# zhyever/Amodal-Depth-Anything

Hardware: AMD Instinct MI355X
Metric: images/sec at 518x518 bs=32 ViT-L (AmodalDAv2 forward) (higher is better)
Workload: dtype f16

## Files before the change

### amodal-depth-anything_amd/csrc/ada_attention.hip

```cpp
#include <stdlib.h>
#include <atomic>
#include <mutex>
#include <type_traits>
#include "ada_common.h"

namespace {

constexpr int HD = 64;
constexpr int QBLK = 128;
constexpr int KVB = 64;
constexpr int ROWB = 128;
constexpr int K_TILE = KVB * ROWB;
constexpr int V_TILE = KVB * ROWB;
constexpr int STAGE = K_TILE + V_TILE;

ADA_DEV void half_exchange(float x, float& lo, float& hi_) {
    unsigned a = __builtin_bit_cast(unsigned, x), b = a;
    asm volatile("s_nop 1\n\tv_permlane32_swap_b32 %0, %1" : "+v"(a), "+v"(b));
    lo = __builtin_bit_cast(float, a);
    hi_ = __builtin_bit_cast(float, b);
}

ADA_DEV float vmax3(float a, float b, float c) {
    float d;
    asm("v_max3_f32 %0, %1, %2, %3" : "=v"(d) : "v"(a), "v"(b), "v"(c));
    return d;
}
ADA_DEV float vmax2(float a, float b) {
    float d;
    asm("v_max_f32 %0, %1, %2" : "=v"(d) : "v"(a), "v"(b));
    return d;
}

struct RowSum {
    float a0 = 0.0f, a1 = 0.0f;
    ADA_DEV void add(float e0, float e1, opx2, bool) {
        a0 += e0;
        a1 += e1;
    }
    ADA_DEV float total() const { return a0 + a1; }
};

__global__ __launch_bounds__(256, 2) void attention_kernel_v3(const op_t* __restrict__ qkv, op_t* __restrict__ out, long ld_out,
                                                           int n_tok, int heads, int nqb, int n_bh) {
    __shared__ __attribute__((aligned(16))) char smem[2 * STAGE];

    const int tid = threadIdx.x;
    const int lane = tid & 63;
    const int wave = __builtin_amdgcn_readfirstlane(tid >> 6);
    const int l31 = lane & 31;
    const int hi = lane >> 5;

    int bh, qb;
    {
        const int nblk = gridDim.x, bid = blockIdx.x;
        const int q = nblk >> 3, r = nblk & 7;
        const int xcd = bid & 7, idx = bid >> 3;
        const int logical = (xcd < r ? xcd * (q + 1) : r * (q + 1) + (xcd - r) * q) + idx;
        bh = logical / nqb;
        qb = logical - bh * nqb;
    }
    const int b = bh / heads, h = bh - b * heads;
    const long D = (long)heads * HD;
    const long row_stride = 3 * D;
    const op_t* base = qkv + (long)b * n_tok * row_stride + (long)h * HD;
    const op_t* qptr = base;
    const op_t* kptr = base + D;
    const op_t* vptr = base + 2 * D;

    const int q_row = qb * QBLK + wave * 32 + l31;
    const int q_ld = q_row < n_tok ? q_row : n_tok - 1;
    const bool wave_active = (qb * QBLK + wave * 32) < n_tok;
    opx8 qf[4];
#pragma unroll
    for (int s = 0; s < 4; ++s) qf[s] = *(const opx8*)(qptr + (long)q_ld * row_stride + 16 * s + 8 * hi);

    const int srow = tid >> 3;
    const int sc = tid & 7;
    const int k_src_chunk = sc ^ ((srow >> 1) & 7);
    const int v_src_chunk = sc ^ (((srow >> 1) & 1) << 2);
    auto stage = [&](int buf, int t) {
        char* dst = smem + buf * STAGE + wave * 1024;
#pragma unroll
        for (int it = 0; it < 2; ++it) {
            int key = t * KVB + it * 32 + srow;
            if (key >= n_tok) key = n_tok - 1;
            const long off = (long)key * row_stride;
            __builtin_amdgcn_global_load_lds((const __attribute__((address_space(1))) void*)(kptr + off + k_src_chunk * 8),
                                             (__attribute__((address_space(3))) void*)(dst + it * 4096), 16, 0, 0);
            __builtin_amdgcn_global_load_lds((const __attribute__((address_space(1))) void*)(vptr + off + v_src_chunk * 8),
                                             (__attribute__((address_space(3))) void*)(dst + K_TILE + it * 4096), 16, 0, 0);
        }
    };

    f32x16 o[2];
#pragma unroll
    for (int db = 0; db < 2; ++db)
#pragma unroll
        for (int r = 0; r < 16; ++r) o[db][r] = 0.0f;
    float m_run = 0.0f, l_run = 0.0f;
    constexpr float RESCALE_THR = 8.0f;

    opx8 kx, qx;
#pragma unroll
    for (int j = 0; j < 8; ++j) { kx[j] = (op_t)0.0f; qx[j] = (op_t)0.0f; }
    if (hi == 0) kx[0] = (op_t)1.0f;

    const unsigned lds0 = (unsigned)(size_t)smem;
    const int swz = (l31 >> 1) & 7;
    unsigned kofs[4];
#pragma unroll
    for (int s = 0; s < 4; ++s) kofs[s] = l31 * ROWB + (((2 * s + hi) ^ swz) * 16);
    const int i16 = lane & 15;
    const int g1 = (lane >> 4) & 1;
    const int vsw = (i16 >> 3) & 1;
    const unsigned v_row_part = (4 * hi + (i16 >> 2)) * ROWB + (16 * g1 + 4 * (i16 & 3)) * 2;
    const unsigned vofs[2] = {v_row_part + (vsw ? 64u : 0u), v_row_part + (vsw ? 0u : 64u)};

    const int nt = (n_tok + KVB - 1) / KVB;
    stage(0, 0);
    asm volatile("s_waitcnt vmcnt(0)" ::: "memory");
    __syncthreads();

    for (int t = 0; t < nt; ++t) {
        const int cur = t & 1;
        if (t + 1 < nt) stage(cur ^ 1, t + 1);
        const unsigned kbase_l = lds0 + cur * STAGE;
        const unsigned vbase0 = kbase_l + K_TILE + vofs[0], vbase1 = kbase_l + K_TILE + vofs[1];

        if (wave_active) {
        opx8 kf[2][4];
#pragma unroll
        for (int kb = 0; kb < 2; ++kb)
#pragma unroll
            for (int s = 0; s < 4; ++s)
                asm volatile("ds_read_b128 %0, %1 offset:%2" : "=v"(kf[kb][s]) : "v"(kbase_l + kofs[s]), "i"(kb * 32 * ROWB));
        asm volatile("s_waitcnt lgkmcnt(0)" ::: "memory");
        __builtin_amdgcn_sched_barrier(0);
        f32x16 sT[2];
#pragma unroll
        for (int kb = 0; kb < 2; ++kb) {
#pragma unroll
            for (int r = 0; r < 16; ++r) sT[kb][r] = 0.0f;
            sT[kb] = mfma32(kx, qx, sT[kb]);
#pragma unroll
            for (int s = 0; s < 4; ++s) sT[kb] = mfma32(kf[kb][s], qf[s], sT[kb]);
        }
        __builtin_amdgcn_sched_barrier(0);
        opx4 vlo[2][2][2], vhi[2][2][2];
#pragma unroll
        for (int kb = 0; kb < 2; ++kb)
#pragma unroll
            for (int s = 0; s < 2; ++s) {
                asm volatile("ds_read_b64_tr_b16 %0, %1 offset:%2" : "=v"(vlo[kb][s][0]) : "v"(vbase0), "i"((kb * 32 + s * 16) * ROWB));
                asm volatile("ds_read_b64_tr_b16 %0, %1 offset:%2" : "=v"(vhi[kb][s][0]) : "v"(vbase0), "i"((kb * 32 + s * 16 + 8) * ROWB));
                asm volatile("ds_read_b64_tr_b16 %0, %1 offset:%2" : "=v"(vlo[kb][s][1]) : "v"(vbase1), "i"((kb * 32 + s * 16) * ROWB));
                asm volatile("ds_read_b64_tr_b16 %0, %1 offset:%2" : "=v"(vhi[kb][s][1]) : "v"(vbase1), "i"((kb * 32 + s * 16 + 8) * ROWB));
            }
        if (t == nt - 1) {
            const int kv0 = t * KVB;
#pragma unroll
            for (int kb = 0; kb < 2; ++kb)
#pragma unroll
                for (int r = 0; r < 16; ++r)
                    if (kv0 + kb * 32 + crow32(r, hi) >= n_tok) sT[kb][r] = -INFINITY;
        }

        float mx = sT[0][0];
#pragma unroll
        for (int kb = 0; kb < 2; ++kb)
#pragma unroll
            for (int r = 0; r < 16; ++r) mx = __builtin_fmaxf(mx, sT[kb][r]);
        {
            float a, b2;
            half_exchange(mx, a, b2);
            mx = __builtin_fmaxf(a, b2);
        }
        if (t == 0 || __any(mx > RESCALE_THR)) {
            const bool mv = (t == 0) || (mx > RESCALE_THR);
            const op_t m16 = (op_t)(m_run + mx);
            const float m_new = mv ? (float)m16 : m_run;
            const float delta = m_new - m_run;
            const float alpha = __builtin_amdgcn_fmed3f(__builtin_amdgcn_exp2f(-delta), 0.0f, 1.0f);
            l_run *= alpha;
            m_run = m_new;
            if (hi == 0) qx[0] = (op_t)(-m_new);
#pragma unroll
            for (int db = 0; db < 2; ++db)
#pragma unroll
                for (int r = 0; r < 16; ++r) o[db][r] *= alpha;
#pragma unroll
            for (int kb = 0; kb < 2; ++kb)
#pragma unroll
                for (int r = 0; r < 16; ++r) sT[kb][r] -= delta;
        }
        opx8 pf[2][2];
        RowSum rs;
#pragma unroll
        for (int kb = 0; kb < 2; ++kb) {
#pragma unroll
            for (int r = 0; r < 16; r += 2) {
                opx2 pp;
                const float e0 = __builtin_amdgcn_exp2f(sT[kb][r]), e1 = __builtin_amdgcn_exp2f(sT[kb][r + 1]);
                pp[0] = (op_t)e0;
                pp[1] = (op_t)e1;
                pf[kb][r >> 3][r & 7] = pp[0];
                pf[kb][r >> 3][(r & 7) + 1] = pp[1];
                rs.add(e0, e1, pp, (r & 2) != 0);
            }
        }
        l_run += rs.total();

        asm volatile("s_waitcnt lgkmcnt(0)" ::: "memory");
        __builtin_amdgcn_sched_barrier(0);
#pragma unroll
        for (int kb = 0; kb < 2; ++kb) {
#pragma unroll
            for (int s = 0; s < 2; ++s) {
#pragma unroll
                for (int db = 0; db < 2; ++db) {
                    const opx4 lo = vlo[kb][s][db], hi4 = vhi[kb][s][db];
                    opx8 vf;
                    vf[0] = lo[0]; vf[1] = lo[1]; vf[2] = lo[2]; vf[3] = lo[3];
                    vf[4] = hi4[0]; vf[5] = hi4[1]; vf[6] = hi4[2]; vf[7] = hi4[3];
                    o[db] = mfma32(vf, pf[kb][s], o[db]);
                }
            }
        }
        __builtin_amdgcn_sched_barrier(0);
        }

        asm volatile("s_waitcnt vmcnt(0)" ::: "memory");
        __syncthreads();
    }

    float l_lo, l_hi;
    half_exchange(l_run, l_lo, l_hi);
    const float inv = 1.0f / (l_lo + l_hi);
    if (q_row < n_tok) {
        op_t* orow = out + ((long)b * n_tok + q_row) * ld_out + (long)h * HD;
#pragma unroll
        for (int db = 0; db < 2; ++db) {
#pragma unroll
            for (int g = 0; g < 4; ++g) {
                opx4 v4;
#pragma unroll
                for (int e = 0; e < 4; ++e) v4[e] = to_op(o[db][g * 4 + e] * inv);
                *(opx4*)(orow + db * 32 + 8 * g + 4 * hi) = v4;
            }
        }
    }
}


#ifndef ADA_ATTN_MFMA_ROWSUM
#define ADA_ATTN_MFMA_ROWSUM 1
#endif
#ifndef ADA_ATTN_OCC
#define ADA_ATTN_OCC 2
#endif
__global__ __launch_bounds__(256, ADA_ATTN_OCC) void attention_kernel_mix(const op_t* __restrict__ qkv, op_t* __restrict__ out, long ld_out,
                                                               int split_seg, int split_f8, int n_tok, int heads, int nqb, int n_bh) {
    __shared__ __attribute__((aligned(16))) char smem[2 * K_TILE + 2 * V_TILE];

    const int tid = threadIdx.x;
    const int lane = tid & 63;
    const int wave = __builtin_amdgcn_readfirstlane(tid >> 6);
    const int l31 = lane & 31;
    const int hi = lane >> 5;

    int bh, qb;
    {
        const int nblk = gridDim.x, bid = blockIdx.x;
        const int q = nblk >> 3, r = nblk & 7;
        const int xcd = bid & 7, idx = bid >> 3;
        const int logical = (xcd < r ? xcd * (q + 1) : r * (q + 1) + (xcd - r) * q) + idx;
        bh = logical / nqb;
        qb = logical - bh * nqb;
    }
    const int b = bh / heads, h = bh - b * heads;
    const long D = (long)heads * HD;
    const long row_stride = 3 * D;
    const op_t* base = qkv + (long)b * n_tok * row_stride + (long)h * HD;

    const unsigned win_bytes = (unsigned)((long)(n_tok - 1) * row_stride * 2 + HD * 2);
    const __amdgpu_buffer_rsrc_t k_rsrc = __builtin_amdgcn_make_buffer_rsrc((void*)(base + D), 0, (int)win_bytes, 0x20000);
    const __amdgpu_buffer_rsrc_t v_rsrc = __builtin_amdgcn_make_buffer_rsrc((void*)(base + 2 * D), 0, (int)win_bytes, 0x20000);

    const int q_row = qb * QBLK + wave * 32 + l31;
    const int q_ld = q_row < n_tok ? q_row : n_tok - 1;
    const bool wave_active = (qb * QBLK + wave * 32) < n_tok;
    opx8 qf[4];
#pragma unroll
    for (int s = 0; s < 4; ++s) qf[s] = *(const opx8*)(base + (long)q_ld * row_stride + 16 * s + 8 * hi);

    const int srow = tid >> 3, sc = tid & 7;
    const unsigned row_bytes = (unsigned)(row_stride * 2);
    const unsigned k_voff = (unsigned)srow * row_bytes + (unsigned)((sc ^ ((srow >> 1) & 7)) * 16);
    const unsigned v_voff = (unsigned)srow * row_bytes + (unsigned)((sc ^ (((srow >> 1) & 1) << 2)) * 16);
    const unsigned pass_bytes = 32u * row_bytes;
    char* const my_lds = smem + wave * 1024;
    auto stage_k = [&](int buf, int tile) {
        const int so = __builtin_amdgcn_readfirstlane((int)((unsigned)tile * 2u * pass_bytes));
        __builtin_amdgcn_raw_ptr_buffer_load_lds(k_rsrc, (__attribute__((address_space(3))) void*)(my_lds + buf * K_TILE), 16, (int)k_voff, so, 0, 0);
        __builtin_amdgcn_raw_ptr_buffer_load_lds(k_rsrc, (__attribute__((address_space(3))) void*)(my_lds + buf * K_TILE + 4096), 16, (int)(k_voff + pass_bytes), so, 0, 0);
    };
    auto stage_v = [&](int buf, int tile) {
        const int so = __builtin_amdgcn_readfirstlane((int)((unsigned)tile * 2u * pass_bytes));
        __builtin_amdgcn_raw_ptr_buffer_load_lds(v_rsrc, (__attribute__((address_space(3))) void*)(my_lds + 2 * K_TILE + buf * V_TILE), 16, (int)v_voff, so, 0, 0);
        __builtin_amdgcn_raw_ptr_buffer_load_lds(v_rsrc, (__attribute__((address_space(3))) void*)(my_lds + 2 * K_TILE + buf * V_TILE + 4096), 16, (int)(v_voff + pass_bytes), so, 0, 0);
    };

    f32x16 o[2], negm, sT[2];
#pragma unroll
    for (int r = 0; r < 16; ++r) { o[0][r] = 0.0f; o[1][r] = 0.0f; negm[r] = 0.0f; }
    float m_run = 0.0f, l_run = 0.0f;
    constexpr float RESCALE_THR = 8.0f;
    constexpr bool MROW = ADA_ATTN_MFMA_ROWSUM != 0;
    f32x4 lacc = {0.0f, 0.0f, 0.0f, 0.0f};
    opx8 sel;
    {
        const int srow_ = lane & 15, kg = lane >> 4;
        const op_t one = (op_t)(((srow_ == 0 && (kg & 1) == 0) || (srow_ == 1 && (kg & 1) == 1)) ? 1.0f : 0.0f);
#pragma unroll
        for (int e = 0; e < 8; ++e) sel[e] = one;
    }

    const unsigned lds0 = (unsigned)(size_t)smem;
    const int swz = (l31 >> 1) & 7;
    unsigned kofs[4];
#pragma unroll
    for (int s = 0; s < 4; ++s) kofs[s] = lds0 + l31 * ROWB + (((2 * s + hi) ^ swz) * 16);
    const int i16 = lane & 15;
    const int g1 = (lane >> 4) & 1;
    const int vsw = (i16 >> 3) & 1;
    const unsigned v_row_part = lds0 + 2 * K_TILE + (4 * hi + (i16 >> 2)) * ROWB + (16 * g1 + 4 * (i16 & 3)) * 2;
    const unsigned vofs0 = v_row_part + (vsw ? 64u : 0u), vofs1 = v_row_part + (vsw ? 0u : 64u);

    const int nt = (n_tok + KVB - 1) / KVB;

    opx8 kf[2][4];
    opx8 vf[2][2][2];
    opx8 pf[2][2], pn[2][2];
#pragma unroll
    for (int kb = 0; kb < 2; ++kb)
#pragma unroll
        for (int s = 0; s < 2; ++s) {
#pragma unroll
            for (int e = 0; e < 8; ++e) { pf[kb][s][e] = (op_t)0.0f; vf[kb][s][0][e] = (op_t)0.0f; vf[kb][s][1][e] = (op_t)0.0f; }
        }

    auto read_v = [&](auto pbuf, int kb, int s, int db) {
        constexpr int PB = decltype(pbuf)::value;
        u32x2 lo, hi2;
        const unsigned a = db ? vofs1 : vofs0;
        if (kb == 0 && s == 0) {
            asm volatile("ds_read_b64_tr_b16 %0, %1 offset:%2" : "=v"(lo) : "v"(a), "i"(PB * V_TILE + (0 * 32 + 0 * 16) * ROWB));
            asm volatile("ds_read_b64_tr_b16 %0, %1 offset:%2" : "=v"(hi2) : "v"(a), "i"(PB * V_TILE + (0 * 32 + 0 * 16 + 8) * ROWB));
        } else if (kb == 0 && s == 1) {
            asm volatile("ds_read_b64_tr_b16 %0, %1 offset:%2" : "=v"(lo) : "v"(a), "i"(PB * V_TILE + (0 * 32 + 1 * 16) * ROWB));
            asm volatile("ds_read_b64_tr_b16 %0, %1 offset:%2" : "=v"(hi2) : "v"(a), "i"(PB * V_TILE + (0 * 32 + 1 * 16 + 8) * ROWB));
        } else if (kb == 1 && s == 0) {
            asm volatile("ds_read_b64_tr_b16 %0, %1 offset:%2" : "=v"(lo) : "v"(a), "i"(PB * V_TILE + (1 * 32 + 0 * 16) * ROWB));
            asm volatile("ds_read_b64_tr_b16 %0, %1 offset:%2" : "=v"(hi2) : "v"(a), "i"(PB * V_TILE + (1 * 32 + 0 * 16 + 8) * ROWB));
        } else {
            asm volatile("ds_read_b64_tr_b16 %0, %1 offset:%2" : "=v"(lo) : "v"(a), "i"(PB * V_TILE + (1 * 32 + 1 * 16) * ROWB));
            asm volatile("ds_read_b64_tr_b16 %0, %1 offset:%2" : "=v"(hi2) : "v"(a), "i"(PB * V_TILE + (1 * 32 + 1 * 16 + 8) * ROWB));
        }
        u32x4 w;
        w[0] = lo[0]; w[1] = lo[1]; w[2] = hi2[0]; w[3] = hi2[1];
        vf[kb][s][db] = __builtin_bit_cast(opx8, w);
    };
    auto read_k = [&](auto pbuf, int kb, int s) {
        constexpr int PB = decltype(pbuf)::value;
        (void)kf; (void)kofs;
        if (kb == 0) asm volatile("ds_read_b128 %0, %1 offset:%2" : "=v"(kf[0][s]) : "v"(kofs[s]), "i"(PB * K_TILE));
        else asm volatile("ds_read_b128 %0, %1 offset:%2" : "=v"(kf[1][s]) : "v"(kofs[s]), "i"(PB * K_TILE + 32 * ROWB));
    };
    RowSum rs;
    float mx0 = 0.0f;
    auto sm_unit = [&](int u) {
        const int kb = u >> 3, r = (u & 7) * 2;
        opx2 pp;
        const float e0 = __builtin_amdgcn_exp2f(sT[kb][r]), e1 = __builtin_amdgcn_exp2f(sT[kb][r + 1]);
        pp[0] = (op_t)e0;
        pp[1] = (op_t)e1;
        pn[kb][r >> 3][r & 7] = pp[0];
        pn[kb][r >> 3][(r & 7) + 1] = pp[1];
        if constexpr (!MROW) rs.add(e0, e1, pp, (r & 2) != 0);
    };
    auto fence = []() { __builtin_amdgcn_sched_barrier(0); };

    stage_k(0, 0);
    stage_v(0, 0);
    stage_k(1, 1);
    asm volatile("s_waitcnt vmcnt(0)" : "+v"(qf[0]), "+v"(qf[1]), "+v"(qf[2]), "+v"(qf[3])::"memory");
    __syncthreads();
    using I0 = std::integral_constant<int, 0>;
    using I1 = std::integral_constant<int, 1>;
#pragma unroll
    for (int kb = 0; kb < 2; ++kb)
#pragma unroll
        for (int s = 0; s < 4; ++s) read_k(I0{}, kb, s);
    asm volatile("s_waitcnt lgkmcnt(0)" ::: "memory");
    fence();
    sT[0] = mfma32(kf[0][0], qf[0], negm);
    sT[1] = mfma32(kf[1][0], qf[0], negm);
#pragma unroll
    for (int s = 1; s < 4; ++s) {
        sT[0] = mfma32(kf[0][s], qf[s], sT[0]);
        sT[1] = mfma32(kf[1][s], qf[s], sT[1]);
    }
    __syncthreads();

    auto iteration = [&](auto parity, int j) {
        constexpr int P = decltype(parity)::value;
        using PB = std::integral_constant<int, P>;
        using PN = std::integral_constant<int, P ^ 1>;
        stage_k(P, j + 2);
        stage_v(P ^ 1, j + 1);
        fence();
        if (wave_active) {
            if (j == nt - 1) {
                asm volatile(";;ADA_RARE_BEGIN last tile: keys >= n_tok masked");
                const int kv0 = j * KVB;
#pragma unroll
                for (int kb = 0; kb < 2; ++kb)
#pragma unroll
                    for (int r = 0; r < 16; ++r)
                        if (kv0 + kb * 32 + crow32(r, hi) >= n_tok) sT[kb][r] = -INFINITY;
                asm volatile(";;ADA_RARE_END");
            }
            if (j == nt - 1 || j == 0) {
                asm volatile(";;ADA_RARE_BEGIN first / last tile: maximum of key block 0 not taken under the previous tile's MFMAs");
                mx0 = vmax2(sT[0][0], sT[0][1]);
#pragma unroll
                for (int r = 2; r < 16; r += 2) mx0 = vmax3(mx0, sT[0][r], sT[0][r + 1]);
                asm volatile(";;ADA_RARE_END");
            }
            float mx1 = vmax3(mx0, sT[1][0], sT[1][1]);
#pragma unroll
            for (int r = 2; r < 16; r += 2) mx1 = vmax3(mx1, sT[1][r], sT[1][r + 1]);
            float mx = mx1;
            {
                float a, b2;
                half_exchange(mx, a, b2);
                mx = vmax2(a, b2);
            }
            if (j == 0 || __any(mx > RESCALE_THR)) {
                asm volatile(";;ADA_RARE_BEGIN deferred rescale (first tile, or a row maximum grew by more than 2^8)");
                const bool mv = (j == 0) || (mx > RESCALE_THR);
                const float m_new = mv ? m_run + mx : m_run;
                const float delta = m_new - m_run;
                const float alpha = __builtin_amdgcn_fmed3f(__builtin_amdgcn_exp2f(-delta), 0.0f, 1.0f);
                const op_t alpha_op = (op_t)alpha;
                if constexpr (MROW) {
                    lacc[0] *= alpha;
                    lacc[1] *= __shfl(alpha, (lane & 15) + 16);
                } else {
                    l_run *= alpha;
                }
                m_run = m_new;
#pragma unroll
                for (int r = 0; r < 16; ++r) negm[r] = -m_new;
#pragma unroll
                for (int db = 0; db < 2; ++db)
#pragma unroll
                    for (int r = 0; r < 16; ++r) o[db][r] *= alpha;
#pragma unroll
                for (int kb = 0; kb < 2; ++kb)
#pragma unroll
                    for (int s = 0; s < 2; ++s)
#pragma unroll
                        for (int e = 0; e < 8; ++e) pf[kb][s][e] = pf[kb][s][e] * alpha_op;
#pragma unroll
                for (int kb = 0; kb < 2; ++kb)
#pragma unroll
                    for (int r = 0; r < 16; ++r) sT[kb][r] -= delta;
                asm volatile(";;ADA_RARE_END");
            }
            rs = RowSum();
            fence();
#pragma unroll
            for (int g = 0; g < 8; ++g) {
                const int kb = g >> 2, s = (g >> 1) & 1, db = g & 1;
                o[db] = mfma32(vf[kb][s][db], pf[kb][s], o[db]);
                if (MROW && db == 1) lacc = mfma16(sel, pf[kb][s], lacc);
                if (g < 4) { sm_unit(2 * g); sm_unit(2 * g + 1); }
                else sm_unit(4 + g);
                if (g < 4) { read_k(PN{}, 0, g); read_k(PN{}, 1, g); }
                fence();
            }
            asm volatile("s_waitcnt lgkmcnt(0)" : "+v"(kf[0][0]), "+v"(kf[0][1]), "+v"(kf[0][2]), "+v"(kf[0][3]), "+v"(kf[1][0]), "+v"(kf[1][1]), "+v"(kf[1][2]), "+v"(kf[1][3]));
            fence();
#pragma unroll
            for (int g = 0; g < 8; ++g) {
                const int kb = g >> 2, s = g & 3;
                if (s == 0) sT[kb] = mfma32(kf[kb][0], qf[0], negm);
                else sT[kb] = mfma32(kf[kb][s], qf[s], sT[kb]);
                if (g < 4) {
                    sm_unit(12 + g);
                    read_v(PB{}, g >> 1, g & 1, 0);
                    read_v(PB{}, g >> 1, g & 1, 1);
                } else {
                    const int r = (g - 4) * 4;
                    mx0 = g == 4 ? vmax2(sT[0][0], sT[0][1]) : vmax3(mx0, sT[0][r], sT[0][r + 1]);
                    mx0 = vmax3(mx0, sT[0][r + 2], sT[0][r + 3]);
                }
                fence();
            }
            if constexpr (!MROW) l_run += rs.total();
#pragma unroll
            for (int kb = 0; kb < 2; ++kb)
#pragma unroll
                for (int s = 0; s < 2; ++s) pf[kb][s] = pn[kb][s];
        }
        asm volatile("s_waitcnt lgkmcnt(0)" : "+v"(vf[0][0][0]), "+v"(vf[0][0][1]), "+v"(vf[0][1][0]), "+v"(vf[0][1][1]), "+v"(vf[1][0][0]), "+v"(vf[1][0][1]), "+v"(vf[1][1][0]), "+v"(vf[1][1][1]));
        asm volatile("s_waitcnt vmcnt(0)" ::: "memory");
        fence();
        __builtin_amdgcn_s_barrier();
        fence();
    };

    for (int j = 0; j < nt; j += 2) {
        iteration(I0{}, j);
        if (j + 1 < nt) iteration(I1{}, j + 1);
    }
    if (wave_active) {
#pragma unroll
        for (int g = 0; g < 8; ++g) {
            const int kb = g >> 2, s = (g >> 1) & 1, db = g & 1;
            o[db] = mfma32(vf[kb][s][db], pf[kb][s], o[db]);
            if (MROW && db == 1) lacc = mfma16(sel, pf[kb][s], lacc);
        }
    }
    float inv;
    if constexpr (MROW) {
        const float s0 = __shfl(lacc[0], lane & 15), s1 = __shfl(lacc[1], lane & 15);
        inv = 1.0f / (((lane & 31) < 16) ? s0 : s1);
    } else {
        float l_lo, l_hi;
        half_exchange(l_run, l_lo, l_hi);
        inv = 1.0f / (l_lo + l_hi);
    }
    op_t* const rowp = out + ((long)b * n_tok + (q_row < n_tok ? q_row : 0)) * ld_out;
    op_t* const orow = rowp + (long)h * HD;
#pragma unroll
    for (int db = 0; db < 2; ++db) {
#pragma unroll
        for (int g = 0; g < 4; g += 2) {
            opx4 va, vb;
            float fa[4], fb[4];
#pragma unroll
            for (int e = 0; e < 4; ++e) {
                fa[e] = o[db][g * 4 + e] * inv;
                fb[e] = o[db][(g + 1) * 4 + e] * inv;
                va[e] = to_op(fa[e]);
                vb[e] = to_op(fb[e]);
            }
            u32x2 a = __builtin_bit_cast(u32x2, va), c = __builtin_bit_cast(u32x2, vb);
            unsigned a0 = a[0], a1 = a[1], c0 = c[0], c1 = c[1];
            asm volatile("s_nop 1\n\tv_permlane32_swap_b32 %0, %1" : "+v"(a0), "+v"(c0));
            asm volatile("s_nop 1\n\tv_permlane32_swap_b32 %0, %1" : "+v"(a1), "+v"(c1));
            const int col = db * 32 + 8 * (g + hi);
            if (q_row < n_tok) *(u32x4*)(orow + col) = u32x4{a0, a1, c0, c1};
            if (split_seg > 0) {
                float ra[4], rb[4];
#pragma unroll
                for (int e = 0; e < 4; ++e) {
                    ra[e] = fa[e] - (float)va[e];
                    rb[e] = fb[e] - (float)vb[e];
                }
                if (split_f8) {
                    unsigned la = bf8x4(ra[0] * ADA_F8_LO_SHIFT, ra[1] * ADA_F8_LO_SHIFT, ra[2] * ADA_F8_LO_SHIFT, ra[3] * ADA_F8_LO_SHIFT);
                    unsigned lb = bf8x4(rb[0] * ADA_F8_LO_SHIFT, rb[1] * ADA_F8_LO_SHIFT, rb[2] * ADA_F8_LO_SHIFT, rb[3] * ADA_F8_LO_SHIFT);
                    unsigned ha = bf8x4(fa[0], fa[1], fa[2], fa[3]), hb = bf8x4(fb[0], fb[1], fb[2], fb[3]);
                    asm volatile("s_nop 1\n\tv_permlane32_swap_b32 %0, %1" : "+v"(la), "+v"(lb));
                    asm volatile("s_nop 1\n\tv_permlane32_swap_b32 %0, %1" : "+v"(ha), "+v"(hb));
                    char* const b8 = (char*)(rowp + split_seg) + (h * HD + col);
                    if (q_row < n_tok) {
                        *(u32x2*)b8 = u32x2{la, lb};
                        *(u32x2*)(b8 + split_seg) = u32x2{ha, hb};
                    }
                } else {
                    opx4 la4, lb4;
#pragma unroll
                    for (int e = 0; e < 4; ++e) {
                        la4[e] = to_op(ra[e]);
                        lb4[e] = to_op(rb[e]);
                    }
                    u32x2 la = __builtin_bit_cast(u32x2, la4), lb = __builtin_bit_cast(u32x2, lb4);
                    unsigned l0 = la[0], l1 = la[1], m0 = lb[0], m1 = lb[1];
                    asm volatile("s_nop 1\n\tv_permlane32_swap_b32 %0, %1" : "+v"(l0), "+v"(m0));
                    asm volatile("s_nop 1\n\tv_permlane32_swap_b32 %0, %1" : "+v"(l1), "+v"(m1));
                    if (q_row < n_tok) *(u32x4*)(orow + split_seg + col) = u32x4{l0, l1, m0, m1};
                }
            }
        }
    }
}

}

static std::atomic<int> g_attn_variant{5};
extern "C" void ada_debug_set_attention_variant(int v) { g_attn_variant.store(v == 3 ? 3 : 5, std::memory_order_relaxed); }

extern "C" int ada_attention_ex(const void* qkv, void* out, int32_t batch, int32_t n_tokens, int32_t heads, int64_t ld_out, int32_t split_seg, void* stream) {
    static std::once_flag env_once;
    std::call_once(env_once, []() {
        const char* e = getenv("ADA_ATTN_VARIANT");
        if (e) ada_debug_set_attention_variant(atoi(e));
    });
    ADA_REQUIRE(qkv && out, ADA_EINVAL, "ada_attention_fwd: null pointer");
    ADA_REQUIRE(batch > 0 && n_tokens > 0 && heads > 0, ADA_EINVAL, "ada_attention_fwd: bad shape B=%d N=%d H=%d", batch, n_tokens, heads);
    ADA_REQUIRE(((uintptr_t)qkv % 16) == 0 && ((uintptr_t)out % 16) == 0, ADA_EINVAL, "ada_attention_fwd: buffers must be 16-byte aligned");
    const long Dm = (long)heads * HD;
    const int seg = split_seg < 0 ? -split_seg : split_seg;
    if (ld_out == 0) ld_out = Dm;
    ADA_REQUIRE(ld_out >= Dm && ld_out % 8 == 0, ADA_EINVAL, "ada_attention_ex: ld_out=%ld must be a multiple of 8 and >= heads * 64", (long)ld_out);
    ADA_REQUIRE(seg == 0 || (seg >= Dm && seg % 8 == 0 && ld_out >= 2L * seg), ADA_EINVAL,
                "ada_attention_ex: split_seg=%d needs |split_seg| >= heads * 64, a multiple of 8, and ld_out >= 2 |split_seg| (ld_out=%ld)", split_seg, (long)ld_out);
    const int nqb = (n_tokens + QBLK - 1) / QBLK;
    const long nblk = (long)nqb * batch * heads;
    ADA_REQUIRE(nblk < (1L << 31), ADA_EUNSUPPORTED, "ada_attention_fwd: grid too large");
    ADA_REQUIRE((long)n_tokens * 3 * heads * HD * 2 < (1L << 31), ADA_EUNSUPPORTED, "ada_attention_fwd: one image's qkv rows exceed the 2 GiB buffer window");
    if (g_attn_variant.load(std::memory_order_relaxed) == 3 && seg == 0)
        hipLaunchKernelGGL(attention_kernel_v3, dim3((unsigned)nblk), dim3(256), 0, (hipStream_t)stream, (const op_t*)qkv, (op_t*)out, (long)ld_out,
                           n_tokens, heads, nqb, batch * heads);
    else
        hipLaunchKernelGGL(attention_kernel_mix, dim3((unsigned)nblk), dim3(256), 0, (hipStream_t)stream, (const op_t*)qkv, (op_t*)out, (long)ld_out,
                           seg, split_seg < 0 ? 1 : 0, n_tokens, heads, nqb, batch * heads);
    return ada_check_launch("ada_attention_fwd");
}

extern "C" int ada_attention_fwd(const void* qkv, void* out, int32_t batch, int32_t n_tokens, int32_t heads, void* stream) {
    return ada_attention_ex(qkv, out, batch, n_tokens, heads, 0, 0, stream);
}
```

Before: 601.5.

## Fix softmax max after first tile with overflow guard and exact fallback

The default attention kernel now takes the exact row maximum only on the first KV tile. Later tiles skip the per-tile max reduction and online rescale, and instead compute a per-tile row sum of P with an MFMA. A guard checks that sum: if it exceeds 2^14 it rescales by a power of two, and if it is inf or NaN it sets a flag so the whole query block is rerun on the exact loop. This cuts VALU max work and rescale branches from the inner loop. The cost is an extra MFMA per tile and the rare full recompute. The previous exact kernel stays available as variant 6.

```diff
diff --git a/amodal-depth-anything_amd/csrc/ada_attention.hip b/amodal-depth-anything_amd/csrc/ada_attention.hip
--- a/amodal-depth-anything_amd/csrc/ada_attention.hip
+++ b/amodal-depth-anything_amd/csrc/ada_attention.hip
@@ -259,9 +259,11 @@
 #ifndef ADA_ATTN_OCC
 #define ADA_ATTN_OCC 2
 #endif
-__global__ __launch_bounds__(256, ADA_ATTN_OCC) void attention_kernel_mix(const op_t* __restrict__ qkv, op_t* __restrict__ out, long ld_out,
-                                                               int split_seg, int split_f8, int n_tok, int heads, int nqb, int n_bh) {
+template <bool EXACT_ONLY>
+ADA_DEV void attention_mix_body(const op_t* __restrict__ qkv, op_t* __restrict__ out, long ld_out,
+                                int split_seg, int split_f8, int n_tok, int heads, int nqb, int n_bh) {
     __shared__ __attribute__((aligned(16))) char smem[2 * K_TILE + 2 * V_TILE];
+    __shared__ int redo_flag;
 
     const int tid = threadIdx.x;
     const int lane = tid & 63;
@@ -312,12 +314,12 @@
     };
 
     f32x16 o[2], negm, sT[2];
-#pragma unroll
-    for (int r = 0; r < 16; ++r) { o[0][r] = 0.0f; o[1][r] = 0.0f; negm[r] = 0.0f; }
-    float m_run = 0.0f, l_run = 0.0f;
+    float m_run, l_run;
     constexpr float RESCALE_THR = 8.0f;
+    constexpr float GUARD_THR = 0x1p14f;
     constexpr bool MROW = ADA_ATTN_MFMA_ROWSUM != 0;
-    f32x4 lacc = {0.0f, 0.0f, 0.0f, 0.0f};
+    f32x4 lacc;
+    f32x4 ltile;
     opx8 sel;
     {
         const int srow_ = lane & 15, kg = lane >> 4;
@@ -342,13 +344,6 @@
     opx8 kf[2][4];
     opx8 vf[2][2][2];
     opx8 pf[2][2], pn[2][2];
-#pragma unroll
-    for (int kb = 0; kb < 2; ++kb)
-#pragma unroll
-        for (int s = 0; s < 2; ++s) {
-#pragma unroll
-            for (int e = 0; e < 8; ++e) { pf[kb][s][e] = (op_t)0.0f; vf[kb][s][0][e] = (op_t)0.0f; vf[kb][s][1][e] = (op_t)0.0f; }
-        }
 
     auto read_v = [&](auto pbuf, int kb, int s, int db) {
         constexpr int PB = decltype(pbuf)::value;
@@ -391,29 +386,93 @@
     };
     auto fence = []() { __builtin_amdgcn_sched_barrier(0); };
 
-    stage_k(0, 0);
-    stage_v(0, 0);
-    stage_k(1, 1);
-    asm volatile("s_waitcnt vmcnt(0)" : "+v"(qf[0]), "+v"(qf[1]), "+v"(qf[2]), "+v"(qf[3])::"memory");
-    __syncthreads();
     using I0 = std::integral_constant<int, 0>;
     using I1 = std::integral_constant<int, 1>;
-#pragma unroll
-    for (int kb = 0; kb < 2; ++kb)
-#pragma unroll
-        for (int s = 0; s < 4; ++s) read_k(I0{}, kb, s);
-    asm volatile("s_waitcnt lgkmcnt(0)" ::: "memory");
-    fence();
-    sT[0] = mfma32(kf[0][0], qf[0], negm);
-    sT[1] = mfma32(kf[1][0], qf[0], negm);
-#pragma unroll
-    for (int s = 1; s < 4; ++s) {
-        sT[0] = mfma32(kf[0][s], qf[s], sT[0]);
-        sT[1] = mfma32(kf[1][s], qf[s], sT[1]);
-    }
-    __syncthreads();
-
-    auto iteration = [&](auto parity, int j) {
+    using Exact = std::integral_constant<bool, true>;
+    using Fast = std::integral_constant<bool, false>;
+
+    auto prologue = [&]() {
+#pragma unroll
+        for (int r = 0; r < 16; ++r) { o[0][r] = 0.0f; o[1][r] = 0.0f; negm[r] = 0.0f; }
+        m_run = 0.0f;
+        l_run = 0.0f;
+        lacc = f32x4{0.0f, 0.0f, 0.0f, 0.0f};
+        ltile = f32x4{0.0f, 0.0f, 0.0f, 0.0f};
+#pragma unroll
+        for (int kb = 0; kb < 2; ++kb)
+#pragma unroll
+            for (int s = 0; s < 2; ++s) {
+#pragma unroll
+                for (int e = 0; e < 8; ++e) { pf[kb][s][e] = (op_t)0.0f; vf[kb][s][0][e] = (op_t)0.0f; vf[kb][s][1][e] = (op_t)0.0f; }
+            }
+        asm volatile("" : "+v"(vf[0][0][0]), "+v"(vf[0][0][1]), "+v"(vf[0][1][0]), "+v"(vf[0][1][1]), "+v"(vf[1][0][0]), "+v"(vf[1][0][1]), "+v"(vf[1][1][0]), "+v"(vf[1][1][1]));
+        asm volatile("" : "+v"(pf[0][0]), "+v"(pf[0][1]), "+v"(pf[1][0]), "+v"(pf[1][1]), "+v"(lacc), "+v"(ltile), "+v"(o[0]), "+v"(o[1]), "+v"(negm));
+        stage_k(0, 0);
+        stage_v(0, 0);
+        stage_k(1, 1);
+        asm volatile("s_waitcnt vmcnt(0)" : "+v"(qf[0]), "+v"(qf[1]), "+v"(qf[2]), "+v"(qf[3])::"memory");
+        __syncthreads();
+#pragma unroll
+        for (int kb = 0; kb < 2; ++kb)
+#pragma unroll
+            for (int s = 0; s < 4; ++s) read_k(I0{}, kb, s);
+        asm volatile("s_waitcnt lgkmcnt(0)" ::: "memory");
+        fence();
+        sT[0] = mfma32(kf[0][0], qf[0], negm);
+        sT[1] = mfma32(kf[1][0], qf[0], negm);
+#pragma unroll
+        for (int s = 1; s < 4; ++s) {
+            sT[0] = mfma32(kf[0][s], qf[s], sT[0]);
+            sT[1] = mfma32(kf[1][s], qf[s], sT[1]);
+        }
+        __syncthreads();
+    };
+
+    auto guard = [&]() {
+        lacc[0] += ltile[0];
+        lacc[1] += ltile[1];
+        if (__any(!(ltile[0] <= GUARD_THR) || !(ltile[1] <= GUARD_THR))) {
+            asm volatile(";;ADA_RARE_BEGIN row-sum guard: some row sum of P is above 2^14, inf or NaN");
+            if (__any(!(ltile[0] < INFINITY) || !(ltile[1] < INFINITY))) {
+                asm volatile(";;ADA_RARE_BEGIN row-sum guard, path B");
+                if (lane == 0) redo_flag = 1;
+                asm volatile(";;ADA_RARE_END");
+            } else {
+                asm volatile(";;ADA_RARE_BEGIN row-sum guard, path A");
+                const int e0 = ltile[0] > GUARD_THR ? __builtin_amdgcn_frexp_expf(ltile[0]) : 0;
+                const int e1 = ltile[1] > GUARD_THR ? __builtin_amdgcn_frexp_expf(ltile[1]) : 0;
+                lacc[0] = __builtin_ldexpf(lacc[0], -e0);
+                lacc[1] = __builtin_ldexpf(lacc[1], -e1);
+                const int d0 = __shfl(e0, lane & 15), d1 = __shfl(e1, lane & 15);
+                const int de = l31 < 16 ? d0 : d1;
+                const float delta = (float)de;
+                const op_t alpha_op = (op_t)__builtin_ldexpf(1.0f, -de);
+                m_run += delta;
+#pragma unroll
+                for (int r = 0; r < 16; ++r) negm[r] -= delta;
+#pragma unroll
+                for (int db = 0; db < 2; ++db)
+#pragma unroll
+                    for (int r = 0; r < 16; ++r) o[db][r] = __builtin_ldexpf(o[db][r], -de);
+#pragma unroll
+                for (int kb = 0; kb < 2; ++kb)
+#pragma unroll
+                    for (int s = 0; s < 2; ++s)
+#pragma unroll
+                        for (int e = 0; e < 8; ++e) pf[kb][s][e] = pf[kb][s][e] * alpha_op;
+#pragma unroll
+                for (int kb = 0; kb < 2; ++kb)
+#pragma unroll
+                    for (int r = 0; r < 16; ++r) sT[kb][r] -= delta;
+                asm volatile(";;ADA_RARE_END");
+            }
+            asm volatile(";;ADA_RARE_END");
+        }
+    };
+
+    auto iteration = [&](auto exact, auto first, auto parity, int j) {
+        constexpr bool EXACT = decltype(exact)::value || !MROW;
+        constexpr bool FIRST = decltype(first)::value;
         constexpr int P = decltype(parity)::value;
         using PB = std::integral_constant<int, P>;
         using PN = std::integral_constant<int, P ^ 1>;
@@ -431,6 +490,10 @@
                         if (kv0 + kb * 32 + crow32(r, hi) >= n_tok) sT[kb][r] = -INFINITY;
                 asm volatile(";;ADA_RARE_END");
             }
+            if constexpr (!EXACT && !FIRST) {
+                guard();
+            } else {
+            if constexpr (!EXACT) asm volatile(";;ADA_RARE_BEGIN fast loop, tile 0: the exact row maximum sets m");
             if (j == nt - 1 || j == 0) {
                 asm volatile(";;ADA_RARE_BEGIN first / last tile: maximum of key block 0 not taken under the previous tile's MFMAs");
                 mx0 = vmax2(sT[0][0], sT[0][1]);
@@ -479,13 +542,15 @@
                     for (int r = 0; r < 16; ++r) sT[kb][r] -= delta;
                 asm volatile(";;ADA_RARE_END");
             }
+            if constexpr (!EXACT) asm volatile(";;ADA_RARE_END");
+            }
             rs = RowSum();
             fence();
 #pragma unroll
             for (int g = 0; g < 8; ++g) {
                 const int kb = g >> 2, s = (g >> 1) & 1, db = g & 1;
                 o[db] = mfma32(vf[kb][s][db], pf[kb][s], o[db]);
-                if (MROW && db == 1) lacc = mfma16(sel, pf[kb][s], lacc);
+                if (MROW && EXACT && db == 1) lacc = mfma16(sel, pf[kb][s], lacc);
                 if (g < 4) { sm_unit(2 * g); sm_unit(2 * g + 1); }
                 else sm_unit(4 + g);
                 if (g < 4) { read_k(PN{}, 0, g); read_k(PN{}, 1, g); }
@@ -502,10 +567,13 @@
                     sm_unit(12 + g);
                     read_v(PB{}, g >> 1, g & 1, 0);
                     read_v(PB{}, g >> 1, g & 1, 1);
-                } else {
+                } else if constexpr (EXACT) {
                     const int r = (g - 4) * 4;
                     mx0 = g == 4 ? vmax2(sT[0][0], sT[0][1]) : vmax3(mx0, sT[0][r], sT[0][r + 1]);
                     mx0 = vmax3(mx0, sT[0][r + 2], sT[0][r + 3]);
+                } else {
+                    const int f = g - 4;
+                    ltile = mfma16(sel, pn[f >> 1][f & 1], f == 0 ? f32x4{0.0f, 0.0f, 0.0f, 0.0f} : ltile);
                 }
                 fence();
             }
@@ -522,16 +590,41 @@
         fence();
     };
 
-    for (int j = 0; j < nt; j += 2) {
-        iteration(I0{}, j);
-        if (j + 1 < nt) iteration(I1{}, j + 1);
-    }
-    if (wave_active) {
-#pragma unroll
-        for (int g = 0; g < 8; ++g) {
-            const int kb = g >> 2, s = (g >> 1) & 1, db = g & 1;
-            o[db] = mfma32(vf[kb][s][db], pf[kb][s], o[db]);
-            if (MROW && db == 1) lacc = mfma16(sel, pf[kb][s], lacc);
+    auto run = [&](auto exact) {
+        constexpr bool EXACT = decltype(exact)::value || !MROW;
+        prologue();
+        if constexpr (EXACT) {
+            for (int j = 0; j < nt; j += 2) {
+                iteration(exact, Fast{}, I0{}, j);
+                if (j + 1 < nt) iteration(exact, Fast{}, I1{}, j + 1);
+            }
+        } else {
+            iteration(exact, Exact{}, I0{}, 0);
+            for (int j = 1; j < nt; j += 2) {
+                iteration(exact, Fast{}, I1{}, j);
+                if (j + 1 < nt) iteration(exact, Fast{}, I0{}, j + 1);
+            }
+        }
+        if (wave_active) {
+            if constexpr (!EXACT) guard();
+#pragma unroll
+            for (int g = 0; g < 8; ++g) {
+                const int kb = g >> 2, s = (g >> 1) & 1, db = g & 1;
+                o[db] = mfma32(vf[kb][s][db], pf[kb][s], o[db]);
+                if (MROW && EXACT && db == 1) lacc = mfma16(sel, pf[kb][s], lacc);
+            }
+        }
+    };
+    if constexpr (EXACT_ONLY || !MROW) {
+        run(Exact{});
+    } else {
+        if (tid == 0) redo_flag = 0;
+        run(Fast{});
+        __syncthreads();
+        if (__builtin_amdgcn_readfirstlane(redo_flag)) {
+            asm volatile(";;ADA_RARE_BEGIN some wave's P overflowed: the whole query block again, on the exact loop");
+            run(Exact{});
+            asm volatile(";;ADA_RARE_END");
         }
     }
     float inv;
@@ -600,10 +693,19 @@
     }
 }
 
+__global__ __launch_bounds__(256, ADA_ATTN_OCC) void attention_kernel_mix(const op_t* __restrict__ qkv, op_t* __restrict__ out, long ld_out,
+                                                               int split_seg, int split_f8, int n_tok, int heads, int nqb, int n_bh) {
+    attention_mix_body<false>(qkv, out, ld_out, split_seg, split_f8, n_tok, heads, nqb, n_bh);
+}
+__global__ __launch_bounds__(256, ADA_ATTN_OCC) void attention_kernel_mix_exact(const op_t* __restrict__ qkv, op_t* __restrict__ out, long ld_out,
+                                                                     int split_seg, int split_f8, int n_tok, int heads, int nqb, int n_bh) {
+    attention_mix_body<true>(qkv, out, ld_out, split_seg, split_f8, n_tok, heads, nqb, n_bh);
+}
+
 }
 
 static std::atomic<int> g_attn_variant{5};
-extern "C" void ada_debug_set_attention_variant(int v) { g_attn_variant.store(v == 3 ? 3 : 5, std::memory_order_relaxed); }
+extern "C" void ada_debug_set_attention_variant(int v) { g_attn_variant.store(v == 3 || v == 6 ? v : 5, std::memory_order_relaxed); }
 
 extern "C" int ada_attention_ex(const void* qkv, void* out, int32_t batch, int32_t n_tokens, int32_t heads, int64_t ld_out, int32_t split_seg, void* stream) {
     static std::once_flag env_once;
@@ -624,9 +726,13 @@
     const long nblk = (long)nqb * batch * heads;
     ADA_REQUIRE(nblk < (1L << 31), ADA_EUNSUPPORTED, "ada_attention_fwd: grid too large");
     ADA_REQUIRE((long)n_tokens * 3 * heads * HD * 2 < (1L << 31), ADA_EUNSUPPORTED, "ada_attention_fwd: one image's qkv rows exceed the 2 GiB buffer window");
-    if (g_attn_variant.load(std::memory_order_relaxed) == 3 && seg == 0)
+    const int variant = g_attn_variant.load(std::memory_order_relaxed);
+    if (variant == 3 && seg == 0)
         hipLaunchKernelGGL(attention_kernel_v3, dim3((unsigned)nblk), dim3(256), 0, (hipStream_t)stream, (const op_t*)qkv, (op_t*)out, (long)ld_out,
                            n_tokens, heads, nqb, batch * heads);
+    else if (variant == 6)
+        hipLaunchKernelGGL(attention_kernel_mix_exact, dim3((unsigned)nblk), dim3(256), 0, (hipStream_t)stream, (const op_t*)qkv, (op_t*)out, (long)ld_out,
+                           seg, split_seg < 0 ? 1 : 0, n_tokens, heads, nqb, batch * heads);
     else
         hipLaunchKernelGGL(attention_kernel_mix, dim3((unsigned)nblk), dim3(256), 0, (hipStream_t)stream, (const op_t*)qkv, (op_t*)out, (long)ld_out,
                            seg, split_seg < 0 ? 1 : 0, n_tokens, heads, nqb, batch * heads);
```

New measurement: 598.4. Within noise of the previous version (-0.5%).
